# PolusAI/nyxus

Hardware: AMD Instinct MI355X
Metric: ROIs/sec (*ALL_GLCM*+*ALL_INTENSITY*, 1024^2 tiles) (higher is better)
Workload: dtype f64; 1 GPU; *ALL_GLCM*+*ALL_INTENSITY*, coarse_gray_depth=8, 4 angles, d=1, 1000 synthetic 1024x1024 tiles/GPU x 196 ROIs/tile (disk r=30, 2821 px, bbox 61x61), intensities U[1,4095]; reduce stage on pre-assembled ROI clouds resident in HBM; n_columns=185

## Files before the change

nyxus_amd/csrc/nyxhip_ctx.h:

```cpp
#pragma once
#include <hip/hip_runtime.h>
#include <math.h>
#include <stdio.h>
#include <stdlib.h>
#include <string.h>
#include <unistd.h>
#include <string>
#include <vector>
#include <algorithm>
#include <atomic>
#include <utility>

#include "../../include/nyxhip.h"
#include "roi_kernel.h"
#include "roi_radial.h"

struct DevBuf {
    void* p = nullptr;
    size_t bytes = 0;
    DevBuf() = default;
    DevBuf(const DevBuf&) = delete;
    DevBuf& operator=(const DevBuf&) = delete;
    DevBuf(DevBuf&& o) noexcept : p(o.p), bytes(o.bytes) { o.p = nullptr; o.bytes = 0; }
    DevBuf& operator=(DevBuf&& o) noexcept
// ... 65 lines not shown
};
constexpr int NYXHIP_INTERNAL_NEEDS_CLOUDS = -1000;

struct nyxhip_ctx {
    int device = 0;
    hipStream_t own_stream = nullptr;
    hipStream_t user_stream = nullptr;
    bool use_user_stream = false;
    DevBuf d_status;
    uint64_t census_small = 0, census_total = 0, census_pending = 0;
    DevBuf d_bank;
    DevBuf d_bank32;
    DevBuf d_bank16;
    std::vector<double> bank_key;
    uint32_t bank_zero_rows[NYXHIP_MAX_GABOR_FILTERS + 1] = {};
    uint32_t bank_lp_sep = 0;
    float bank_lp_B[16] = {}, bank_lp_C[44] = {};
    uint32_t bank_box_mask = 0;
    DevBuf d_stamps;
    std::string err;
    DevBuf d_stage;
    DevBuf d_glcm_ws;
    DevBuf d_glcm_ng;
    DevBuf d_logtab;
    uint32_t logtab_n = 0;
    DevBuf d_mom;
    DevBuf d_spill_list;
    DevBuf d_spill;
    DevBuf d_tile;
    DevBuf d_cloud;
    DevBuf d_slot[2];
    hipStream_t copy_stream = nullptr;
    hipEvent_t slot_ready[2] = {nullptr, nullptr}, slot_free[2] = {nullptr, nullptr};
    static constexpr int kStageSlots = 4;
    static constexpr size_t kStageSlotBytes = (size_t)32 << 20;
    PinnedSlot h_stage[kStageSlots];
    int h_stage_next = 0;
    nyxhip::WindowSrc win_next = {};
    uint32_t tile_cap_hint = 0;
    DevBuf d_res;
    size_t res_cap = 0, res_rows = 0, res_cols = 0;
    double* res_table() const { return d_res.as<double>(); }
    uint32_t* res_label() const { return (uint32_t*)(d_res.as<char>() + (((size_t)res_cap * res_cols * 8 + 255) & ~(size_t)255)); }
    uint32_t* res_tile() const { return res_label() + res_cap; }
    DevBuf d_cls_list;
    DevBuf d_cls_hdr;
// ... 53 lines not shown
```

nyxus_amd/csrc/nyxhip_dispatch.hip:

```cpp
#include "nyxhip_ctx.h"

using namespace nyxhip;

namespace {

uint32_t align16(uint32_t v) { return (v + 15u) & ~15u; }

void gabor_filter(double* Gex, double f0, double sig2lam, double gamma, double theta, double fi, int n)
{
    const double lambda = 2 * M_PI / f0, cos_theta = cos(theta), sin_theta = sin(theta), sig = sig2lam * lambda;
    std::vector<double> tx(n + 1), ty(n + 1);
    tx[0] = (n % 2 > 0) ? -((n - 1) / 2) : -(n / 2);
    for (int x = 1; x < n; x++) tx[x] = tx[x - 1] + 1;
    ty[0] = tx[0];
    for (int y = 1; y < n; y++) ty[y] = ty[y - 1] + 1;
    double sum = 0;
    for (int y = 0; y < n; y++)
        for (int x = 0; x < n; x++) {
            double xte = tx[x] * cos_theta + ty[y] * sin_theta;
            double yte = ty[y] * cos_theta - tx[x] * sin_theta;
            double rte = xte * xte + gamma * gamma * yte * yte;
            double ge = exp(-1 * rte / (2 * sig * sig));
            double argm = xte * f0 + fi;
            int idx = y * n * 2 + x * 2;
// ... 272 lines not shown
    int c_glrlm = n_cols1, c_gldzm = c_glrlm + ((mask & NYXHIP_FAM_GLRLM) ? kGlrlmCols : 0);
    int c_glszm = c_gldzm + ((mask & NYXHIP_FAM_GLDZM) ? kGldzmCols : 0), c_gldm = c_glszm + ((mask & NYXHIP_FAM_GLSZM) ? kGlszmCols : 0);
    int c_ngldm = c_gldm + ((mask & NYXHIP_FAM_GLDM) ? kGldmCols : 0);
    if (mask1 && (groups & 1)) {
        if (int lrc = make_layout(mask1, s, n_cols1, E.px, E.area, E.range, a.L, why, cap, E.vmax, E.wide_only))
            return lrc;
        a.n_roi = b->n_roi;
        a.px_offset = b->px_offset; a.x = b->x; a.y = b->y; a.inten = b->inten;
        a.bbox_w = b->bbox_w; a.bbox_h = b->bbox_h; a.min_inten = b->min_inten; a.max_inten = b->max_inten;
        a.slide_min = b->slide_min; a.slide_max = b->slide_max;
        a.out = d_out; a.ld = ld; a.status = ctx->d_status.as<int>();
        a.stamps = ctx->d_stamps.as<unsigned long long>();
        if (cap == 0) a.win = ctx->win_next;
        a.mask = mask1; a.n_cols = n_cols1;
        int c = 0;
        a.col_intensity = a.col_glcm = -1;
        if (mask1 & NYXHIP_FAM_INTENSITY) { a.col_intensity = c; c += kIntensityCols; }
        if (mask1 & NYXHIP_FAM_GLCM) { a.col_glcm = c; c += kGlcmAngled * s->glcm_n_angles + kGlcmAve; }
        a.soft_nan = s->soft_nan;
        a.grey_depth = s->grey_depth; a.ibsi = s->ibsi; a.glcm_grey_depth = s->glcm_grey_depth;
        a.glcm_offset = s->glcm_offset; a.glcm_na = s->glcm_n_angles; a.glcm_symmetric = s->glcm_symmetric;
        for (int i = 0; i < kMaxAngles; i++) a.glcm_angles[i] = s->glcm_angles[i];
        a.n_hist = abs(s->grey_depth);
        const int gi = s->ibsi ? 0 : s->grey_depth;
        if ((mask1 & NYXHIP_FAM_GLCM) && cap == 0 && gi >= 0 && a.L.ng_cap <= 16 && (int)a.L.app >= s->glcm_n_angles && s->glcm_n_angles > 0) {
            const size_t stride = (size_t)s->glcm_n_angles * a.L.ng_cap * a.L.ng_cap;
            const size_t need = 4 * stride * (size_t)b->n_roi + 256;
            if (ctx->d_glcm_ws.reserve(need, nullptr) != hipSuccess || !ctx->d_glcm_ng) {
                why = "out of device memory for the GLCM count workspace";
                return NYXHIP_ERR_HIP;
            }
            {
                a.glcm_ng = ctx->d_glcm_ng.as<uint32_t>();
                a.glcm_ws = ctx->d_glcm_ws.as<uint32_t>();
                a.glcm_ws_stride = (uint32_t)stride;
            }
        }
    }
    if (mask2 && (groups & 2)) {
        if (int lrc = make_tex_layout(mask2, s, n_cols2, E.area, E.side, t.L, why, cap, E.vmax))
            return lrc;
        t.n_roi = b->n_roi;
        t.px_offset = b->px_offset; t.x = b->x; t.y = b->y; t.inten = b->inten;
        t.bbox_w = b->bbox_w; t.bbox_h = b->bbox_h; t.min_inten = b->min_inten; t.max_inten = b->max_inten;
        t.out = d_out; t.ld = ld; t.status = ctx->d_status.as<int>();
        t.mask = mask2; t.n_cols = n_cols2; t.col0 = n_cols1;
// ... 740 lines not shown
        if (int brc = ensure_gabor_bank(ctx, s))
            return brc;
    hipStream_t st = ctx->stream();
    const uint32_t n_roi = (uint32_t)b->n_roi;
    clear_runs(ctx);
    if (!ctx->lane_fork) HIP_TRY(ctx, hipEventCreateWithFlags(&ctx->lane_fork, hipEventDisableTiming));
    HIP_TRY(ctx, hipEventRecord(ctx->lane_fork, st));
    struct LaneJoin {
        nyxhip_ctx* c; hipStream_t st;
        ~LaneJoin() {
            for (int k = 0; k < nyxhip_ctx::kLanes; k++)
                if (c->lane_used[k]) {
                    (void)hipEventRecord(c->lane_done[k], c->lane_stream[k]);
                    (void)hipStreamWaitEvent(st, c->lane_done[k], 0);
                    c->lane_used[k] = false;
                }
        }
    } lane_join{ctx, st};
    if (mask & NYXHIP_FAM_GLCM) {
        const size_t need = 4ull * n_roi + 256;
        HIP_TRY(ctx, ctx->d_glcm_ng.reserve(need, st, need + need / 4));
        HIP_TRY(ctx, hipMemsetAsync(ctx->d_glcm_ng.p, 0, 4ull * n_roi, st));
    }
    auto timed_class = [&](int cls, uint32_t count, const Extrema& E, const uint32_t* lp, uint32_t grid, uint32_t class_mask = 0, uint32_t group_sel = 0xF,
                           const ClassTotals* tot = nullptr) -> int {
        ClassRun r{cls, count, E, 0, nullptr, nullptr};
        if (ctx->timing >= 2) {
            HIP_TRY(ctx, hipEventCreate(&r.e0));
            HIP_TRY(ctx, hipEventCreate(&r.e1));
            HIP_TRY(ctx, hipEventRecord(r.e0, st));
        }
        const int rc = run_class(ctx, b, mask, s, d_out, ld, E, lp, grid, false, nullptr, &r, class_mask, group_sel, cls, tot);
        if (ctx->timing >= 2 && rc == 0) HIP_TRY(ctx, hipEventRecord(r.e1, st));
        ctx->runs.push_back(r);
        return rc;
    };
    if ((mask & ~kContourFams) || !hinted) {
        bool done = false;
        static const bool force_exact = [] { const char* e = getenv("NYXHIP_CLASS_SYNC"); return e && *e && *e != '0'; }();
        const bool need_vmax = s->ibsi && (mask & (NYXHIP_FAM_GLCM | kTexture | kDependence));
        const bool wide_possible = max_range >= 16384u && (mask & NYXHIP_FAM_INTENSITY);
        const bool has_m1 = !(max_px <= kClassPx[0] && max_side <= kClassSide[0]);
        static const bool no_small = [] { const char* e = getenv("NYXHIP_NO_SMALL"); return e && *e && *e != '0'; }();
        static const bool no_adapt = [] { const char* e = getenv("NYXHIP_NO_ADAPT"); return e && *e && *e != '0'; }();
        const bool small_fits = !no_small && ((mask & NYXHIP_FAM_INTENSITY) || (!s->ibsi && s->grey_depth > 0 && s->grey_depth <= 64));
        const bool two_filtered = (mask & (NYXHIP_FAM_INTENSITY | NYXHIP_FAM_GLCM)) && has_m1 && small_fits;
// ... 339 lines not shown
```

nyxus_amd/csrc/roi_features.hip:

```cpp
#include <hip/hip_runtime.h>
#include <type_traits>
#include <algorithm>
#include <cstdlib>
#include <cstdio>
#include "device_math.h"
#include "roi_kernel.h"
#include "launch_util.h"
#include "glcm_rows.h"
#include "glcm_w64.h"
#include "sort_lds.h"
#include "../../include/nyxhip.h"

namespace nyxhip {


enum { S_MEAN = 0, S_P10, S_P90, S_MEDIAN, S_MODE, S_NG };


template <int NW> __device__ __forceinline__ double xw_chain(const double* s_red, int k)
{
    return NW == 1 ? s_red[k] : ((s_red[k] + s_red[8 + k]) + s_red[16 + k]) + s_red[24 + k];
}
template <int NW> __device__ __forceinline__ double xw_pairs(const double* s_red, int k)
{
// ... 654 lines not shown
#define STAMP(i) do { } while (0)
#endif

typedef __attribute__((address_space(3))) uint8_t lds_u8_t;

typedef const __attribute__((address_space(4))) RoiArgs KArgs;
__device__ __forceinline__ KArgs* late_kernarg()
{
    KArgs* p = (KArgs*)__builtin_amdgcn_kernarg_segment_ptr();
    asm volatile("" : "+s"(p));
    return p;
}
template <bool LATE>
struct KView {
    const RoiArgs& a;
    KArgs* p;
    __device__ __forceinline__ explicit KView(const RoiArgs& a_) : a(a_), p(LATE ? late_kernarg() : nullptr) {}
    __device__ __forceinline__ auto operator->() const
    {
        if constexpr (LATE) return p;
        else return &a;
    }
};
template <bool GS, bool C16, bool SPLIT, bool D8, int FAM = 0, int TIER = 4, bool G16 = false, int WIN = 2, int NW = 4>
__device__ __forceinline__ void roi_features_body(const RoiArgs& A, const uint64_t slot)
{
    static_assert((NW == 4 && NW == kMaxAngles) || (NW == 8 && G16 && FAM == 4), "one workgroup of four waves per ROI (and a wave per GLCM angle)");
    constexpr int BS = NW * 64;
    extern __shared__ __attribute__((aligned(16))) unsigned char lds_raw[];
    unsigned char* const lds = GS ? A.sp.scratch + (size_t)blockIdx.x * A.sp.stride : lds_raw;
    const int tid = (int)threadIdx.x, lane = tid & 63, wave = __builtin_amdgcn_readfirstlane(tid >> 6);
    uint64_t roi;
    if (!roi_of_slot(A.sp, slot, A.n_roi, roi))
        return;

    auto reg = [&](uint32_t o) -> unsigned char* { return (GS && o < A.L.gs_lds_bytes) ? lds_raw + o : lds + o; };
    double* s_red = (double*)reg(A.L.red);
    double* s_stat = (double*)reg(A.L.stat);
    uint32_t* s_lb100 = (uint32_t*)reg(A.L.lb100);
    uint32_t* s_lbc = (uint32_t*)reg(A.L.lbc);
    uint32_t* s_val = (uint32_t*)(lds + A.L.val);
    using dense_t = typename std::conditional<D8, uint8_t, uint16_t>::type;
    dense_t* s_dense = (dense_t*)(lds + (D8 ? 0u : A.L.dense));
    uint16_t* s_lvlmap = (uint16_t*)reg(A.L.lvlmap);
    uint32_t* s_P = (uint32_t*)reg(A.L.P);
    double* s_g = (double*)reg(A.L.gscr);

// ... 314 lines not shown
    }

    STAMP(1);
    const KView<FAM != 0 || G16> B(A);
    double* const out_row_l = B->out + roi * B->ld;
    if (do_int) {
        double* o = out_row_l + B->col_intensity;
        const double dn = (double)n;
        if ((unsigned long long)n * vmax < (1ull << 32))
            sum = wave_sum_t<uint32_t>((uint32_t)sum);
        else
            sum = wave_sum_u64(sum);
        if (C16) {
            const uint32_t lo24 = wave_sum_t<uint32_t>((uint32_t)sumsq & 0xFFFFFFu), hi = wave_sum_t<uint32_t>((uint32_t)(sumsq >> 24));
            sumsq = ((unsigned long long)hi << 24) + lo24;
        } else
            sumsq = wave_sum_u64(sumsq);
        if (lane == 0) {
            s_red[wave * 8 + 0] = (double)sum;
            s_red[wave * 8 + 1] = (double)sumsq;
        }
        grp_sync<GS, NW>();
        const bool blank = (vmin == 0 && vmax == 0);
        if (tid == 0) {
            double tot = 0, totsq = 0;
            for (int wv = 0; wv < NW; wv++) {
                tot += s_red[wv * 8 + 0];
                totsq += s_red[wv * 8 + 1];
            }
            const double mean = tot / dn;
            s_stat[S_MEAN] = mean;
            if (FAST)
                s_stat[S_NG] = bin_pixel(vmin, vmin, vmax, B->glcm_grey_depth) == bin_pixel(vmax, vmin, vmax, B->glcm_grey_depth) ? 1.0 : 0.0;
            o[I_MIN] = (double)vmin;
            o[I_MAX] = (double)vmax;
            o[I_RANGE] = (double)vmax - (double)vmin;
            if (B->slide_min && B->slide_max)
                o[I_COVERED_IMAGE_INTENSITY_RANGE] = (double)(vmax - vmin) / (B->slide_max[roi] - B->slide_min[roi]);
            o[I_MEAN] = mean;
            o[I_ENERGY] = totsq;
            o[I_ROOT_MEAN_SQUARED] = sqrt(totsq / dn);
            o[I_INTEGRATED_INTENSITY] = tot;
            if (!blank)
                o[I_UNIFORMITY_PIU] = (1.0 - (double)(vmax - vmin) / (double)(uint32_t)(vmax + vmin)) * 100.0;
        }
        grp_sync<GS, NW>();
        const double mean = s_stat[S_MEAN];
        STAMP(2);

        const double binW100 = (double)range / 100.;
        const uint32_t nb = (uint32_t)B->n_hist;
        auto idx100 = [=](uint32_t v) -> int {
            double realIdx = (double)(v - vmin) / binW100;
            return (realIdx != realIdx) ? 0 : (int)realIdx;
        };

        const uint32_t Q = ((range + 1 + NW * 512 - 1) / (NW * 512)) * 512;
        uint32_t* const s_woff = (uint32_t*)(s_stat + 8);
        if (use_count) {
            uint32_t carry = 0, best_c = 0, best_i = 0;
            const uint32_t base = wave * Q;
            if (C16) {
                uint32_t kk[8] = {0, 0, 0, 0, 0, 0, 0, 0};
                uint32_t inv = 0xFFFFu - (base + 8u * (uint32_t)lane);
                uint4* src = (uint4*)((uint16_t*)s_cnt + base + 8u * (uint32_t)lane);
                uint32_t i = base + 8u * (uint32_t)lane;
                for (uint32_t t = 0; t < Q; t += 512, i += 512, inv -= 512, src += 64) {
// ... 240 lines not shown
                for (int q = 0; q < 6; q++) {
                    const double frac = q == 0 ? 0.01 : q == 1 ? 0.1 : q == 2 ? 0.25 : q == 3 ? 0.75 : q == 4 ? 0.9 : 0.99;
                    const double cnt_p = dn * frac;
                    bool m0 = (double)r0 <= cnt_p && cnt_p <= (double)e0;
                    bool m1 = i1 < 100 && (double)r1 <= cnt_p && cnt_p <= (double)e1;
                    unsigned long long b0 = __ballot(m0), b1 = __ballot(m1);
                    int win = b1 ? 64 + (63 - __clzll((long long)b1)) : (b0 ? 63 - __clzll((long long)b0) : -1);
                    if (lane == q) { mywin = win; mycnt = cnt_p; }
                }
                double pv = 0;
                if (mywin >= 0) {
                    uint32_t rs = s_lb100[mywin], bi = (mywin < 99 ? s_lb100[mywin + 1] : n) - rs;
                    pv = (mycnt - (double)rs) * binW100 / (double)bi + (double)vmin + binW100 * (double)mywin;
                }
                double pq[6];
#pragma unroll
                for (int q = 0; q < 6; q++) {
                    const unsigned long long u = (unsigned long long)__double_as_longlong(pv);
                    const uint32_t lo = (uint32_t)__builtin_amdgcn_readlane((int)(uint32_t)u, q), hi = (uint32_t)__builtin_amdgcn_readlane((int)(uint32_t)(u >> 32), q);
                    pq[q] = __longlong_as_double((long long)(((unsigned long long)hi << 32) | lo));
                }
                if (lane == 0) {
                    o[I_P01] = pq[0]; o[I_P10] = pq[1]; o[I_P25] = pq[2]; o[I_P75] = pq[3]; o[I_P90] = pq[4]; o[I_P99] = pq[5];
                    o[I_QCOD] = (pq[3] - pq[2]) / (pq[3] + pq[2]);
                    o[I_INTERQUARTILE_RANGE] = pq[3] - pq[2];
                    s_stat[S_P10] = pq[1];
                    s_stat[S_P90] = pq[4];
                    if (FUSED) {
                        const double p10 = pq[1], p90 = pq[4];
                        uint32_t lox = 0x80000000u, span = 0;
                        if (p10 <= p90 && p90 >= (double)vmin && p10 <= (double)vmax) {
                            const double cl = ceil(p10), fl = floor(p90);
                            const uint32_t lo_v = cl <= (double)vmin ? vmin : (uint32_t)cl, hi_v = fl >= (double)vmax ? vmax : (uint32_t)fl;
                            if (lo_v <= hi_v) { lox = lo_v - vmin; span = hi_v - lo_v; }
                        }
                        const bool empty = span == 0 && lox == 0x80000000u;
                        uint32_t* const s_rob = (uint32_t*)(s_stat + 6);
                        s_rob[0] = lox;
                        s_rob[1] = span;
                        s_rob[2] = (empty || lox == 0) ? 0u : cum(lox - 1);
                        s_rob[3] = empty ? 0u : cum(lox + span);
                    }
                }
            }
            if (NW == 1 || wave == 1) {
                double e = 0, u = 0;
                for (uint32_t k = lane; k < nb; k += 64) {
                    uint32_t ck = (k < nb - 1 ? s_lbc[k + 1] : n) - s_lbc[k];
// ... 79 lines not shown
                    px1(pv[n_full * BS]);
                {
                    const uint32_t wsx = wave_sum_t<uint32_t>(sx), wsad = wave_sum_t<uint32_t>(sad);
                    if (lane == 0) {
                        s_red[wave * 8 + 6] = (double)wsx;
                        s_red[wave * 8 + 7] = (double)wsad;
                    }
                }
                {
                    double t[8];
#pragma unroll
                    for (int k = 0; k < 8; k++) t[k] = k < 6 ? acc[k] : 0.0;
                    const double tot = wave_transpose_sum8(t, lane);
                    if ((lane & 7) == 0 && (lane >> 3) < 6)
                        s_red[wave * 8 + (lane >> 3)] = tot;
                }
                grp_sync<GS, NW>();
                const uint32_t n_below = (uint32_t)__builtin_amdgcn_readfirstlane((int)s_rob[2]);
                const uint32_t n_upto = (uint32_t)__builtin_amdgcn_readfirstlane((int)s_rob[3]);
                const uint32_t K = n_upto - n_below, n_above = n - n_upto;
                const uint32_t Sx_all = (uint32_t)xw_pairs<NW>(s_red, 6);
                const uint32_t Sxu = (uint32_t)__builtin_amdgcn_readfirstlane((int)(Sx_all - n_below * lox - n_above * hix));
                const double Sx = (double)Sxu, dK = (double)K;
                if (tid == 0) {
                    double a6[6];
#pragma unroll
                    for (int k = 0; k < 6; k++) {
                        a6[k] = xw_chain<NW>(s_red, k);
                        asm volatile("" : "+v"(a6[k]) :: "memory");
                    }
                    const double sadk = xw_pairs<NW>(s_red, 7);
                    const double sadt = 2.0 * sadk + ((m2x & 1u) ? 2.0 * (double)((const uint32_t*)(s_stat + 10))[1] - dn : 0.0);
                    central_outputs(a6);
                    o[I_ROBUST_MEAN] = K ? (Sx + dK * (double)vmin) / dK : 0.0;
                    o[I_MEDIAN_ABSOLUTE_DEVIATION] = fdiv(sadt * 0.5, dn);
                }
                const uint32_t Ku = K;
                const bool fast32 = (unsigned long long)(n_full + 1) * Ku * (span + 1ull) < (1ull << 32);
                double ad1[1];
                if (fast32) {
                    uint32_t ad = 0;
                    auto px2 = [&](uint32_t x) {
                        const uint32_t t = mul_u24_su(med3_u32_ss(x, lox, hix), Ku);
                        asm("v_sad_u32 %0, %1, %2, %0" : "+v"(ad) : "v"(t), "s"(Sxu));
                    };
                    {
                        uint32_t k = 0;
                        for (; k + 1 < n_full; k += 2) { px2(pv[k * BS]); px2(pv[(k + 1) * BS]); }
                        if (k < n_full) px2(pv[k * BS]);
                    }
                    if ((uint32_t)tid < n_rem)
                        px2(pv[n_full * BS]);
                    ad1[0] = (double)ad;
                } else {
                    unsigned long long ad = 0;
                    auto px2 = [&](uint32_t x) {
                        const uint32_t t = (uint32_t)__umul24(Ku, x);
                        uint32_t dlt;
                        asm("v_sad_u32 %0, %1, %2, 0" : "=v"(dlt) : "v"(t), "s"(Sxu));
                        ad += (x - lox) <= span ? dlt : 0u;
                    };
                    for (uint32_t k = 0; k < n_full; k++)
                        px2(pv[k * BS]);
                    if ((uint32_t)tid < n_rem)
                        px2(pv[n_full * BS]);
                    ad1[0] = (double)ad;
                }
                block_sum<1, GS, NW>(ad1, (double*)s_lb100, tid);
                if (tid == 0) {
                    double adin = ad1[0];
                    if (fast32) {
                        const double klo = (double)Ku * (double)lox, khi = (double)Ku * (double)hix;
                        adin -= (double)n_below * fabs(klo - Sx) + (double)n_above * fabs(khi - Sx);
                    }
                    o[I_ROBUST_MEAN_ABSOLUTE_DEVIATION] = K ? fdiv(fdiv(adin, dK), dK) : 0.0;
                }
            } else {
            double rb[3] = {0, 0, 0};
            for (uint32_t i = tid; i < n; i += BS) {
                double a = (double)(C16 ? vmin + ((const uint16_t*)s_val)[i] : SV(i));
                if (a >= p10 && a <= p90) {
                    rb[0] += a;
                    rb[1] += 1.0;
                }
                rb[2] += fabs(a - median);
            }
            block_sum<3, GS, NW>(rb, s_red, tid);
            const double mean1090 = rb[1] > 0 ? rb[0] / rb[1] : 0.0;
            double ad[1] = {0};
            for (uint32_t i = tid; i < n; i += BS) {
                double a = (double)(C16 ? vmin + ((const uint16_t*)s_val)[i] : SV(i));
// ... 144 lines not shown
#pragma unroll
                    for (int q = 0; q < kMaxAngles; q++) {
                        if (q >= na)
                            break;
                        const int ang = B->glcm_angles[q];
                        const int dx = ang == 90 ? 0 : ang == 135 ? -B->glcm_offset : B->glcm_offset, dy = ang == 0 ? 0 : B->glcm_offset;
                        const int r2 = row + dy, c2 = col + dx;
                        if (r2 < 0 || r2 >= (int)h || c2 < 0 || c2 >= (int)w)
                            continue;
                        const uint32_t la = s_dense[(uint32_t)r2 * w + (uint32_t)c2];
                        if (la == 0)
                            continue;
                        atomicAdd(&s_P[q * NN + ((int)lb - 1) * Ng + (int)la - 1], 1u);
                        if (symmetric)
                            atomicAdd(&s_P[q * NN + ((int)la - 1) * Ng + (int)lb - 1], 1u);
                    }
                }
        }
        grp_sync<GS, NW>();
        STAMP(11);
        {
            uint32_t* dst = B->glcm_ws + roi * B->glcm_ws_stride;
            if (dpp) {
                const float inv_nn = __builtin_amdgcn_rcpf((float)NN), inv_ng = __builtin_amdgcn_rcpf((float)Ng);
                for (int i = tid; i < na * NN; i += BS) {
                    const uint32_t q = (uint32_t)(((float)i + 0.5f) * inv_nn), rem = (uint32_t)i - mul24(q, (uint32_t)NN);
                    const uint32_t r = (uint32_t)(((float)rem + 0.5f) * inv_ng), c = rem - mul24(r, (uint32_t)Ng);
                    dst[i] = s_P[mad24(q, (uint32_t)cells, mad24(r + 1u, (uint32_t)NG1, c + 1u))];
                }
            } else
                for (int i = tid; i < na * NN; i += BS)
                    dst[i] = s_P[i];
        }
        STAMP(12);
    } else
    if (do_glcm) {
        double* o = out_row_l + B->col_glcm;
        const int na = B->glcm_na;
        const int ncol_g = kGlcmAngled * na + kGlcmAve;
        const uint32_t vmin_g = (uint32_t)__builtin_amdgcn_readfirstlane((int)vmin), vmax_g = (uint32_t)__builtin_amdgcn_readfirstlane((int)vmax);
        const bool degenerate = bin_pixel(vmin_g, vmin_g, vmax_g, B->glcm_grey_depth) == bin_pixel(vmax_g, vmin_g, vmax_g, B->glcm_grey_depth);

        double* s_I = s_g;
        double* s_f = s_g + B->L.ng_cap;
        double* s_scr = s_f + kMaxAngles * 32;
        if (FAST) {
        } else if (greyInfo > 0) {
            if (tid == 0)
                s_stat[S_NG] = (double)greyInfo;
        } else {
            lvl_max = wave_max_u32(lvl_max);
// ... 514 lines not shown
__global__ __launch_bounds__(kBlock, 4) void roi_features_kernel(const RoiArgs A)
{
    roi_features_body<GS, C16, SPLIT, D8>(A, blockIdx.x);
}

template <bool C16, bool SPLIT, bool D8>
__global__ __launch_bounds__(kBlock, 5) void roi_features_kernel_occ5(const RoiArgs A)
{
    roi_features_body<false, C16, SPLIT, D8, 0, 5>(A, blockIdx.x);
}
template <bool C16, bool SPLIT, bool D8>
__global__ __launch_bounds__(kBlock, 6) void roi_features_kernel_occ6(const RoiArgs A)
{
    roi_features_body<false, C16, SPLIT, D8, 0, 6>(A, blockIdx.x);
}
template <bool C16, bool SPLIT, bool D8>
__global__ __launch_bounds__(kBlock, 7) void roi_features_kernel_occ7(const RoiArgs A)
{
    roi_features_body<false, C16, SPLIT, D8, 0, 7>(A, blockIdx.x);
}
template <int FAM, int WIN>
__global__ __launch_bounds__(kBlock, 8) void roi_features_kernel_occ8(const RoiArgs A)
{
    roi_features_body<false, true, FAM == 1 || FAM == 3, true, FAM, 8, false, WIN>(A, (WIN == 1 && A.win.xcd_swz) ? xcd_slot(blockIdx.x, gridDim.x) : (uint64_t)blockIdx.x);
}
template <int FAM, int WIN>
__global__ __launch_bounds__(kBlock, 7) void roi_features_kernel_fam7(const RoiArgs A)
{
    roi_features_body<false, true, FAM == 1 || FAM == 3, true, FAM, 7, false, WIN>(A, (WIN == 1 && A.win.xcd_swz) ? xcd_slot(blockIdx.x, gridDim.x) : (uint64_t)blockIdx.x);
}
template <int FAM, int WIN>
__global__ __launch_bounds__(kBlock, 6) void roi_features_kernel_fam6(const RoiArgs A)
{
    roi_features_body<false, true, FAM == 1 || FAM == 3, true, FAM, 6, false, WIN>(A, (WIN == 1 && A.win.xcd_swz) ? xcd_slot(blockIdx.x, gridDim.x) : (uint64_t)blockIdx.x);
}

template <int WIN>
__global__ __launch_bounds__(kBlock, 4) void roi_features_kernel_g16(const RoiArgs A)
{
    roi_features_body<false, true, false, true, 0, 9, true, WIN>(A, (WIN == 1 && A.win.xcd_swz) ? xcd_slot(blockIdx.x, gridDim.x) : (uint64_t)blockIdx.x);
}

template <int WIN>
__global__ __launch_bounds__(512, 8) void roi_features_kernel_g16w8(const RoiArgs A)
{
    roi_features_body<false, true, false, true, 4, 9, true, WIN, 8>(A, (WIN == 1 && A.win.xcd_swz) ? xcd_slot(blockIdx.x, gridDim.x) : (uint64_t)blockIdx.x);
}
// ... 98 lines not shown
    for (int q = 0; q < 2; q++) {
        if (Ng[q] == 0) continue;
        double* o = A.out + roi[q] * A.ld + A.col_glcm;
        const double* fq = (const double*)(base + (size_t)q * cnt_bytes);
        for (int c = lane; c < kGlcmAngled * na; c += 64) {
            const int k = sh >= 0 ? c >> sh : c / na, a = c - k * na;
            o[c] = fq[a * 32 + k];
        }
        for (int j = lane; j < kGlcmAve; j += 64) {
            const int k = c_glcm_ave_order[j];
            double init = 0.0;
            int a = 0;
            for (; na - a >= 4; a += 4) {
                const double v1 = fq[a * 32 + k] + fq[(a + 1) * 32 + k];
                const double v2 = fq[(a + 2) * 32 + k] + fq[(a + 3) * 32 + k];
                init = init + (v1 + v2);
            }
            for (; a < na; a++) init = init + fq[a * 32 + k];
            o[kGlcmAngled * na + j] = na == 4 ? init * 0.25 : na == 2 ? init * 0.5 : na ? init / (double)na : 0.0;
        }
    }
}

size_t glcm_features8_lds(uint32_t ng_cap)
{
    return (2 * glcm8_cnt_bytes(ng_cap) + 8ull * (2 * kMaxAngles * 16 + 2 * kMaxAngles * 32)) * kWaves;
}

size_t glcm_features_lds(uint32_t ng_cap)
{
    const size_t per_wave = (((size_t)4 * kMaxAngles * ng_cap * ng_cap + 15) & ~(size_t)15) + 8ull * (ng_cap + kMaxAngles * 6 * ng_cap + 2 * kMaxAngles * 32);
    return per_wave * kWaves;
}

size_t roi_features_max_lds()
{
    return 160 * 1024;
}

namespace {

int no_static_lds(const void* f)
{
    hipFuncAttributes at;
    if (hipError_t e = hipFuncGetAttributes(&at, f); e != hipSuccess)
        return (int)e;
    return at.sharedSizeBytes == 0 ? 0 : (int)hipErrorInvalidConfiguration;
}

template <bool C16, bool SPLIT, bool D8>
int launch_lds_variant(const RoiArgs& a, hipStream_t st, uint32_t grid)
{
    static DeviceOnce optin;
    if (int orc = optin.run([]() -> int {
        const void* fns[22] = {(const void*)roi_features_kernel<false, C16, SPLIT, D8>, (const void*)roi_features_kernel_occ5<C16, SPLIT, D8>,
                               (const void*)roi_features_kernel_occ6<C16, SPLIT, D8>, (const void*)roi_features_kernel_occ7<C16, SPLIT, D8>,
                               (const void*)roi_features_kernel_occ8<1, 0>, (const void*)roi_features_kernel_occ8<2, 0>,
                               (const void*)roi_features_kernel_occ8<1, 1>, (const void*)roi_features_kernel_occ8<2, 1>,
                               (const void*)roi_features_kernel_fam7<1, 0>, (const void*)roi_features_kernel_fam7<2, 0>,
                               (const void*)roi_features_kernel_fam7<1, 1>, (const void*)roi_features_kernel_fam7<2, 1>,
                               (const void*)roi_features_kernel_fam6<1, 0>, (const void*)roi_features_kernel_fam6<2, 0>,
                               (const void*)roi_features_kernel_fam6<1, 1>, (const void*)roi_features_kernel_fam6<2, 1>,
                               (const void*)roi_features_kernel_occ8<3, 0>, (const void*)roi_features_kernel_occ8<3, 1>,
                               (const void*)roi_features_kernel_fam7<3, 0>, (const void*)roi_features_kernel_fam7<3, 1>,
                               (const void*)roi_features_kernel_fam6<3, 0>, (const void*)roi_features_kernel_fam6<3, 1>};
        for (const void* f : fns) {
            hipError_t e = hipFuncSetAttribute(f, hipFuncAttributeMaxDynamicSharedMemorySize, (int)roi_features_max_lds());
            if (e != hipSuccess)
                return (int)e;
            if (int src = no_static_lds(f))
                return src;
        }
        return 0;
    }))
        return orc;
    const size_t lds = roi_features_max_lds();
    const bool int_only = !(a.mask & NYXHIP_FAM_GLCM) && (a.mask & NYXHIP_FAM_INTENSITY);
    const bool int_glcm = (a.mask & NYXHIP_FAM_GLCM) && (a.mask & NYXHIP_FAM_INTENSITY) && a.L.dense8 && a.glcm_ws != nullptr && !a.ibsi &&
                          a.grey_depth > 0 && a.grey_depth <= 16;
    const bool glcm_only = (a.mask & NYXHIP_FAM_GLCM) && !(a.mask & NYXHIP_FAM_INTENSITY) && a.L.dense8 && a.glcm_ws != nullptr && !a.ibsi &&
                           a.grey_depth > 0 && a.grey_depth <= 16;
    const bool fam_ok = C16 && SPLIT && D8 && (int_only || int_glcm || glcm_only);
    int occ = 4;
    for (int o = fam_ok ? 8 : 7; o > 4; o--)
        if ((size_t)o * a.L.total <= lds) { occ = o; break; }
    if (const char* e = getenv("NYXHIP_MAX_OCC")) occ = occ < atoi(e) ? occ : (atoi(e) < 4 ? 4 : atoi(e));
    const bool win = a.win.inten != nullptr;
    if (win && a.win.xcd_swz) grid = (grid + 7u) & ~7u;
    if (fam_ok && glcm_only && occ >= 6) {
        if (occ == 8) { if (win) hipLaunchKernelGGL((roi_features_kernel_occ8<3, 1>), dim3(grid), dim3(kBlock), a.L.total, st, a);
                        else hipLaunchKernelGGL((roi_features_kernel_occ8<3, 0>), dim3(grid), dim3(kBlock), a.L.total, st, a); }
        else if (occ == 7) { if (win) hipLaunchKernelGGL((roi_features_kernel_fam7<3, 1>), dim3(grid), dim3(kBlock), a.L.total, st, a);
                             else hipLaunchKernelGGL((roi_features_kernel_fam7<3, 0>), dim3(grid), dim3(kBlock), a.L.total, st, a); }
        else { if (win) hipLaunchKernelGGL((roi_features_kernel_fam6<3, 1>), dim3(grid), dim3(kBlock), a.L.total, st, a);
               else hipLaunchKernelGGL((roi_features_kernel_fam6<3, 0>), dim3(grid), dim3(kBlock), a.L.total, st, a); }
    }
    else if (occ == 8 && int_only && win) hipLaunchKernelGGL((roi_features_kernel_occ8<2, 1>), dim3(grid), dim3(kBlock), a.L.total, st, a);
    else if (occ == 8 && int_only) hipLaunchKernelGGL((roi_features_kernel_occ8<2, 0>), dim3(grid), dim3(kBlock), a.L.total, st, a);
    else if (occ == 8 && win) hipLaunchKernelGGL((roi_features_kernel_occ8<1, 1>), dim3(grid), dim3(kBlock), a.L.total, st, a);
    else if (occ == 8) hipLaunchKernelGGL((roi_features_kernel_occ8<1, 0>), dim3(grid), dim3(kBlock), a.L.total, st, a);
    else if (fam_ok && occ == 7 && int_only && win) hipLaunchKernelGGL((roi_features_kernel_fam7<2, 1>), dim3(grid), dim3(kBlock), a.L.total, st, a);
    else if (fam_ok && occ == 7 && int_only) hipLaunchKernelGGL((roi_features_kernel_fam7<2, 0>), dim3(grid), dim3(kBlock), a.L.total, st, a);
    else if (fam_ok && occ == 7 && win) hipLaunchKernelGGL((roi_features_kernel_fam7<1, 1>), dim3(grid), dim3(kBlock), a.L.total, st, a);
    else if (fam_ok && occ == 7) hipLaunchKernelGGL((roi_features_kernel_fam7<1, 0>), dim3(grid), dim3(kBlock), a.L.total, st, a);
    else if (fam_ok && occ == 6 && int_only && win) hipLaunchKernelGGL((roi_features_kernel_fam6<2, 1>), dim3(grid), dim3(kBlock), a.L.total, st, a);
    else if (fam_ok && occ == 6 && int_only) hipLaunchKernelGGL((roi_features_kernel_fam6<2, 0>), dim3(grid), dim3(kBlock), a.L.total, st, a);
    else if (fam_ok && occ == 6 && win) hipLaunchKernelGGL((roi_features_kernel_fam6<1, 1>), dim3(grid), dim3(kBlock), a.L.total, st, a);
    else if (fam_ok && occ == 6) hipLaunchKernelGGL((roi_features_kernel_fam6<1, 0>), dim3(grid), dim3(kBlock), a.L.total, st, a);
    else if (occ == 7) hipLaunchKernelGGL((roi_features_kernel_occ7<C16, SPLIT, D8>), dim3(grid), dim3(kBlock), a.L.total, st, a);
    else if (occ == 6) hipLaunchKernelGGL((roi_features_kernel_occ6<C16, SPLIT, D8>), dim3(grid), dim3(kBlock), a.L.total, st, a);
    else if (occ == 5) hipLaunchKernelGGL((roi_features_kernel_occ5<C16, SPLIT, D8>), dim3(grid), dim3(kBlock), a.L.total, st, a);
// ... 23 lines not shown
                for (const void* f : {(const void*)roi_features_kernel_g16<0>, (const void*)roi_features_kernel_g16<1>,
                                      (const void*)roi_features_kernel_g16w8<0>, (const void*)roi_features_kernel_g16w8<1>}) {
                    if (hipError_t e = hipFuncSetAttribute(f, hipFuncAttributeMaxDynamicSharedMemorySize, (int)roi_features_max_lds()); e != hipSuccess)
                        return (int)e;
                    if (int src = no_static_lds(f))
                        return src;
                }
                return 0;
            }))
            return orc;
        static const bool w4 = [] { const char* e = getenv("NYXHIP_G16_W4"); return e && *e && *e != '0'; }();
        static const uint32_t g16_w8_min = [] { const char* e = getenv("NYXHIP_G16_W8_MIN"); return e && *e ? (uint32_t)atoi(e) : 48u * 48u; }();
        if (!(a.mask & NYXHIP_FAM_INTENSITY) && !w4 && a.L.dense_cap >= g16_w8_min) {
            if (a.win.inten != nullptr) hipLaunchKernelGGL(roi_features_kernel_g16w8<1>, dim3(a.win.xcd_swz ? (grid + 7u) & ~7u : grid), dim3(512), a.L.total, st, a);
            else hipLaunchKernelGGL(roi_features_kernel_g16w8<0>, dim3(grid), dim3(512), a.L.total, st, a);
        } else
        if (a.win.inten != nullptr) hipLaunchKernelGGL(roi_features_kernel_g16<1>, dim3(a.win.xcd_swz ? (grid + 7u) & ~7u : grid), dim3(kBlock), a.L.total, st, a);
        else hipLaunchKernelGGL(roi_features_kernel_g16<0>, dim3(grid), dim3(kBlock), a.L.total, st, a);
        return (int)hipGetLastError();
    }
    const bool split = a.glcm_ws != nullptr;
    const bool d8 = a.L.dense8 != 0 || (c16 && !(a.mask & NYXHIP_FAM_GLCM));
    int rc;
    if (a.small_class && !no_small && (c16 || !(a.mask & NYXHIP_FAM_INTENSITY)) && roi_small_supported(a)) rc = launch_roi_small(a, st, grid, a.small_class == 2);
    else
    rc = d8 ? launch_lds_variant<true, true, true>(a, st, grid)
           : c16 ? (split ? launch_lds_variant<true, true, false>(a, st, grid) : launch_lds_variant<true, false, false>(a, st, grid))
                 : (split ? launch_lds_variant<false, true, false>(a, st, grid) : launch_lds_variant<false, false, false>(a, st, grid));
    if (rc == 0 && split && a.glcm_feats != 1) {
        static const bool no_pairs = [] { const char* e = getenv("NYXHIP_GLCM_NO_PAIRS"); return e && *e && *e != '0'; }();
        RoiArgs af = a;
        if (a.glcm_feats == 2) af.sp.class_mask = 0;
        if (a.L.ng_cap <= 8 && !no_pairs)
            hipLaunchKernelGGL(glcm_features_kernel8, dim3((grid + 2 * kWaves - 1) / (2 * kWaves)), dim3(kBlock), glcm_features8_lds(a.L.ng_cap), st, af);
        else
            hipLaunchKernelGGL(glcm_features_kernel, dim3((grid + kWaves - 1) / kWaves), dim3(kBlock), glcm_features_lds(a.L.ng_cap), st, af);
        rc = (int)hipGetLastError();
    }
    return rc;
}

}
```

nyxus_amd/csrc/roi_kernel.h:

```cpp
#pragma once
#include <stdint.h>
#include <stddef.h>
#include "../../include/nyxhip.h"

namespace nyxhip {

constexpr int kBlock = 256;
constexpr int kWaves = kBlock / 64;
constexpr int kIntensityCols = 36;
constexpr int kGlcmAngled = 30;
constexpr int kGlcmAve = 29;
constexpr int kMaxAngles = 4;

constexpr int kSizeClasses = 5, kClasses = 2 * kSizeClasses;
constexpr uint32_t kClassPx[kSizeClasses - 1] = {256, 4096, 16384, 32768};
constexpr uint32_t kClassSide[kSizeClasses - 1] = {32, 64, 128, 256};
constexpr uint32_t kLdsLevels = 128;
constexpr int kFirstLargeSizeClass = 3;
__host__ __device__ inline int roi_class(uint32_t n, uint32_t w, uint32_t h, uint32_t range, uint32_t lvl = 0)
{
    const uint32_t side = w > h ? w : h;
    int sc = (n <= 256u && side <= 32u) ? 0 : (n <= 4096u && side <= 64u) ? 1 : (n <= 16384u && side <= 128u) ? 2 : (n <= 32768u && side <= 256u) ? 3 : 4;
    if (sc == 2 && range >= 65536u) sc = 3;
    if (sc < 3 && lvl > kLdsLevels) sc = 3;
// ... 49 lines not shown
    uint32_t dense_cap;
    uint32_t ng_cap;
    uint32_t lvl_cap;
    uint32_t app;
    uint32_t g16;
    uint32_t gs_lds_bytes;
    uint32_t radix;
    uint32_t radix_k16;
};

struct WindowSrc {
    const void* inten;
    const void* lab;
    int32_t dt_inten, dt_label;
    uint32_t W, H;
    const uint32_t* tile;
    const uint32_t* label;
    const uint32_t* x0;
    const uint32_t* y0;
    uint32_t xcd_swz;
};
__host__ __device__ inline uint64_t xcd_slot(uint32_t b, uint32_t grid) { const uint32_t per = (grid + 7u) >> 3; return (uint64_t)(b & 7u) * per + (b >> 3); }

struct RoiArgs {
    uint64_t n_roi;
    const uint64_t* px_offset;
    const uint16_t* x;
    const uint16_t* y;
    const uint32_t* inten;
    const uint32_t* bbox_w;
    const uint32_t* bbox_h;
    const uint32_t* min_inten;
    const uint32_t* max_inten;
    const double* slide_min;
    const double* slide_max;
    double* out;
    uint64_t ld;
    int* status;
    unsigned long long* stamps;
    uint32_t mask;
    int32_t n_cols;
    int32_t col_intensity;
    int32_t col_glcm;
    double soft_nan;
    int32_t grey_depth, ibsi, glcm_grey_depth, glcm_offset, glcm_na, glcm_symmetric;
    int32_t glcm_angles[kMaxAngles];
    int32_t n_hist;
    uint32_t* glcm_ws;
    uint32_t* glcm_ng;
    uint32_t glcm_ws_stride;
    uint32_t* census;
    uint32_t small_class;
    uint32_t glcm_feats;
    SpillArgs sp;
    WindowSrc win;
    LdsLayout L;
};

constexpr int kGlrlmCols = 16 * 4 + 16;
constexpr int kGlszmCols = 16;
constexpr int kNgtdmCols = 5;

constexpr int kRlmLdsCols = 16;
struct TexLayout {
    uint32_t out;
    uint32_t red;
    uint32_t stat;
    uint32_t dense;
    uint32_t lvlmap;
    uint32_t lv;
    uint32_t lvf;
    uint32_t work;
    uint32_t total;
    uint32_t dense_cap, side_cap, lvl_cap, ng_cap, hash_cap, work_bytes, szm_ok;
    uint32_t szm_c16;
    uint32_t szm_small, szm_smalltab;
// ... 402 lines not shown
```

Measured before the change: 96.99 million ROIs/s.

## Defer intensity feature finalization to a separate close kernel with coalesced writes

In the occupancy-8 fused ROI kernel, intensity scalar epilogues (moments, robust stats, QCOD) are no longer computed and written per ROI. Instead the raw accumulators go into a compact per-ROI record, and a new 64-lane close kernel finishes the math and writes the columns, staged through LDS so stores are spread across lanes. This is meant to shorten the serial tid==0 tail in the main kernel and cut its register and store pressure. The cost is an extra launch plus record and flag traffic. Separately, the GLCM workspace copy uses shift and mask indexing when Ng is a power of two, replacing float reciprocal division.

```diff
diff --git a/nyxus_amd/csrc/nyxhip_ctx.h b/nyxus_amd/csrc/nyxhip_ctx.h
--- a/nyxus_amd/csrc/nyxhip_ctx.h
+++ b/nyxus_amd/csrc/nyxhip_ctx.h
@@ -111,6 +111,8 @@
     DevBuf d_stage;
     DevBuf d_glcm_ws;
     DevBuf d_glcm_ng;
+    DevBuf d_close_rec;
+    DevBuf d_close_flag;
     DevBuf d_logtab;
     uint32_t logtab_n = 0;
     DevBuf d_mom;
diff --git a/nyxus_amd/csrc/nyxhip_dispatch.hip b/nyxus_amd/csrc/nyxhip_dispatch.hip
--- a/nyxus_amd/csrc/nyxhip_dispatch.hip
+++ b/nyxus_amd/csrc/nyxhip_dispatch.hip
@@ -318,6 +318,10 @@
         a.glcm_offset = s->glcm_offset; a.glcm_na = s->glcm_n_angles; a.glcm_symmetric = s->glcm_symmetric;
         for (int i = 0; i < kMaxAngles; i++) a.glcm_angles[i] = s->glcm_angles[i];
         a.n_hist = abs(s->grey_depth);
+        if ((mask1 & NYXHIP_FAM_INTENSITY) && cap == 0) {
+            a.close_rec = ctx->d_close_rec.as<double>();
+            a.close_flag = ctx->d_close_flag.as<uint32_t>();
+        }
         const int gi = s->ibsi ? 0 : s->grey_depth;
         if ((mask1 & NYXHIP_FAM_GLCM) && cap == 0 && gi >= 0 && a.L.ng_cap <= 16 && (int)a.L.app >= s->glcm_n_angles && s->glcm_n_angles > 0) {
             const size_t stride = (size_t)s->glcm_n_angles * a.L.ng_cap * a.L.ng_cap;
@@ -1104,6 +1108,12 @@
         HIP_TRY(ctx, ctx->d_glcm_ng.reserve(need, st, need + need / 4));
         HIP_TRY(ctx, hipMemsetAsync(ctx->d_glcm_ng.p, 0, 4ull * n_roi, st));
     }
+    if (mask & NYXHIP_FAM_INTENSITY) {
+        const size_t need_rec = 8ull * kCloseRec * n_roi + 256, need_flag = 4ull * n_roi + 256;
+        HIP_TRY(ctx, ctx->d_close_rec.reserve(need_rec, st, need_rec + need_rec / 4));
+        HIP_TRY(ctx, ctx->d_close_flag.reserve(need_flag, st, need_flag + need_flag / 4));
+        HIP_TRY(ctx, hipMemsetAsync(ctx->d_close_flag.p, 0, 4ull * n_roi, st));
+    }
     auto timed_class = [&](int cls, uint32_t count, const Extrema& E, const uint32_t* lp, uint32_t grid, uint32_t class_mask = 0, uint32_t group_sel = 0xF,
                            const ClassTotals* tot = nullptr) -> int {
         ClassRun r{cls, count, E, 0, nullptr, nullptr};
diff --git a/nyxus_amd/csrc/roi_features.hip b/nyxus_amd/csrc/roi_features.hip
--- a/nyxus_amd/csrc/roi_features.hip
+++ b/nyxus_amd/csrc/roi_features.hip
@@ -700,7 +700,7 @@
         else return &a;
     }
 };
-template <bool GS, bool C16, bool SPLIT, bool D8, int FAM = 0, int TIER = 4, bool G16 = false, int WIN = 2, int NW = 4>
+template <bool GS, bool C16, bool SPLIT, bool D8, int FAM = 0, int TIER = 4, bool G16 = false, int WIN = 2, int NW = 4, bool DEFER_P = false>
 __device__ __forceinline__ void roi_features_body(const RoiArgs& A, const uint64_t slot)
 {
     static_assert((NW == 4 && NW == kMaxAngles) || (NW == 8 && G16 && FAM == 4), "one workgroup of four waves per ROI (and a wave per GLCM angle)");
@@ -1061,6 +1061,13 @@
         }
         grp_sync<GS, NW>();
         const bool blank = (vmin == 0 && vmax == 0);
+#if defined(NYX_NO_FUSED) || defined(NYX_NO_DEFER)
+        constexpr bool DEFER = false;
+#else
+        constexpr bool DEFER = DEFER_P && C16 && !GS;
+#endif
+        const bool defer = DEFER && !blank;
+        double* const rec = DEFER ? B->close_rec + roi * kCloseRec : nullptr;
         if (tid == 0) {
             double tot = 0, totsq = 0;
             for (int wv = 0; wv < NW; wv++) {
@@ -1071,6 +1078,10 @@
             s_stat[S_MEAN] = mean;
             if (FAST)
                 s_stat[S_NG] = bin_pixel(vmin, vmin, vmax, B->glcm_grey_depth) == bin_pixel(vmax, vmin, vmax, B->glcm_grey_depth) ? 1.0 : 0.0;
+            if (defer) {
+                rec[CR_TOT] = tot;
+                rec[CR_TOTSQ] = totsq;
+            } else {
             o[I_MIN] = (double)vmin;
             o[I_MAX] = (double)vmax;
             o[I_RANGE] = (double)vmax - (double)vmin;
@@ -1082,6 +1093,7 @@
             o[I_INTEGRATED_INTENSITY] = tot;
             if (!blank)
                 o[I_UNIFORMITY_PIU] = (1.0 - (double)(vmax - vmin) / (double)(uint32_t)(vmax + vmin)) * 100.0;
+            }
         }
         grp_sync<GS, NW>();
         const double mean = s_stat[S_MEAN];
@@ -1368,8 +1380,10 @@
                 }
                 if (lane == 0) {
                     o[I_P01] = pq[0]; o[I_P10] = pq[1]; o[I_P25] = pq[2]; o[I_P75] = pq[3]; o[I_P90] = pq[4]; o[I_P99] = pq[5];
-                    o[I_QCOD] = (pq[3] - pq[2]) / (pq[3] + pq[2]);
-                    o[I_INTERQUARTILE_RANGE] = pq[3] - pq[2];
+                    if (!DEFER) {
+                        o[I_QCOD] = (pq[3] - pq[2]) / (pq[3] + pq[2]);
+                        o[I_INTERQUARTILE_RANGE] = pq[3] - pq[2];
+                    }
                     s_stat[S_P10] = pq[1];
                     s_stat[S_P90] = pq[4];
                     if (FUSED) {
@@ -1495,6 +1509,15 @@
                 const uint32_t Sx_all = (uint32_t)xw_pairs<NW>(s_red, 6);
                 const uint32_t Sxu = (uint32_t)__builtin_amdgcn_readfirstlane((int)(Sx_all - n_below * lox - n_above * hix));
                 const double Sx = (double)Sxu, dK = (double)K;
+                if (DEFER) {
+                    if (tid < 8)
+                        rec[CR_ACC + tid] = xw_chain<NW>(s_red, tid);
+                    if (tid == 0) {
+                        uint32_t* const rw = (uint32_t*)rec;
+                        *(uint4*)(rw + CR_W_NBELOW) = make_uint4(n_below, n_above, K, Sxu);
+                        *(uint4*)(rw + CR_W_LOX) = make_uint4(lox, hix, m2x, ((const uint32_t*)(s_stat + 10))[1]);
+                    }
+                } else
                 if (tid == 0) {
                     double a6[6];
 #pragma unroll
@@ -1540,6 +1563,13 @@
                     ad1[0] = (double)ad;
                 }
                 block_sum<1, GS, NW>(ad1, (double*)s_lb100, tid);
+                if (DEFER) {
+                    if (tid == 0) {
+                        rec[CR_ADIN] = ad1[0];
+                        ((uint32_t*)rec)[CR_W_FAST32] = fast32 ? 1u : 0u;
+                        B->close_flag[roi] = 1u;
+                    }
+                } else
                 if (tid == 0) {
                     double adin = ad1[0];
                     if (fast32) {
@@ -1730,11 +1760,21 @@
         {
             uint32_t* dst = B->glcm_ws + roi * B->glcm_ws_stride;
             if (dpp) {
+                if ((Ng & (Ng - 1)) == 0 && ((na * NN) & (BS - 1)) == 0) {
+                    const int lg = 31 - __builtin_clz((unsigned)Ng);
+                    const uint32_t cm = (uint32_t)Ng - 1u;
+                    for (int i0 = 0; i0 < na * NN; i0 += BS) {
+                        const uint32_t i = (uint32_t)(i0 + tid);
+                        const uint32_t q = i >> (2 * lg), r = (i >> lg) & cm, c = i & cm;
+                        dst[i] = s_P[mad24(q, (uint32_t)cells, mad24(r + 1u, (uint32_t)NG1, c + 1u))];
+                    }
+                } else {
                 const float inv_nn = __builtin_amdgcn_rcpf((float)NN), inv_ng = __builtin_amdgcn_rcpf((float)Ng);
                 for (int i = tid; i < na * NN; i += BS) {
                     const uint32_t q = (uint32_t)(((float)i + 0.5f) * inv_nn), rem = (uint32_t)i - mul24(q, (uint32_t)NN);
                     const uint32_t r = (uint32_t)(((float)rem + 0.5f) * inv_ng), c = rem - mul24(r, (uint32_t)Ng);
                     dst[i] = s_P[mad24(q, (uint32_t)cells, mad24(r + 1u, (uint32_t)NG1, c + 1u))];
+                }
                 }
             } else
                 for (int i = tid; i < na * NN; i += BS)
@@ -2295,7 +2335,7 @@
 template <int FAM, int WIN>
 __global__ __launch_bounds__(kBlock, 8) void roi_features_kernel_occ8(const RoiArgs A)
 {
-    roi_features_body<false, true, FAM == 1 || FAM == 3, true, FAM, 8, false, WIN>(A, (WIN == 1 && A.win.xcd_swz) ? xcd_slot(blockIdx.x, gridDim.x) : (uint64_t)blockIdx.x);
+    roi_features_body<false, true, FAM == 1 || FAM == 3, true, FAM, 8, false, WIN, 4, FAM == 1 || FAM == 2>(A, (WIN == 1 && A.win.xcd_swz) ? xcd_slot(blockIdx.x, gridDim.x) : (uint64_t)blockIdx.x);
 }
 template <int FAM, int WIN>
 __global__ __launch_bounds__(kBlock, 7) void roi_features_kernel_fam7(const RoiArgs A)
@@ -2440,6 +2480,137 @@
     }
 }
 
+constexpr int kCloseBlock = 64;
+constexpr uint64_t kCloseCols =
+    (1ull << I_MIN) | (1ull << I_MAX) | (1ull << I_RANGE) | (1ull << I_COVERED_IMAGE_INTENSITY_RANGE) | (1ull << I_MEAN) | (1ull << I_ENERGY) |
+    (1ull << I_ROOT_MEAN_SQUARED) | (1ull << I_INTEGRATED_INTENSITY) | (1ull << I_UNIFORMITY_PIU) | (1ull << I_MEAN_ABSOLUTE_DEVIATION) |
+    (1ull << I_VARIANCE) | (1ull << I_VARIANCE_BIASED) | (1ull << I_STANDARD_DEVIATION) | (1ull << I_STANDARD_DEVIATION_BIASED) | (1ull << I_COV) |
+    (1ull << I_STANDARD_ERROR) | (1ull << I_SKEWNESS) | (1ull << I_KURTOSIS) | (1ull << I_EXCESS_KURTOSIS) | (1ull << I_HYPERSKEWNESS) |
+    (1ull << I_HYPERFLATNESS) | (1ull << I_ROBUST_MEAN) | (1ull << I_MEDIAN_ABSOLUTE_DEVIATION) | (1ull << I_ROBUST_MEAN_ABSOLUTE_DEVIATION) |
+    (1ull << I_QCOD) | (1ull << I_INTERQUARTILE_RANGE);
+__global__ __launch_bounds__(kCloseBlock) void intensity_close_kernel(const RoiArgs A)
+{
+    constexpr int kPitch = __builtin_popcountll(kCloseCols);
+#ifndef NYX_CLOSE_DIRECT
+    __shared__ double s_o[kCloseBlock * kPitch];
+#endif
+    const int lane = (int)threadIdx.x;
+    uint64_t roi = 0;
+    bool mine = roi_of_slot(A.sp, (uint64_t)blockIdx.x * kCloseBlock + (uint64_t)lane, A.n_roi, roi) && glcm_roi_in_launch(A, roi);
+    if (mine) mine = A.close_flag[roi] != 0;
+    const unsigned long long todo = __ballot(mine);
+    if (todo == 0)
+        return;
+#ifdef NYX_CLOSE_DIRECT
+    double* const o = A.out + roi * A.ld + A.col_intensity;
+    auto O = [&](int c) -> double& { return o[c]; };
+#else
+    double* const o = s_o + lane * kPitch;
+    auto O = [&](int c) -> double& { return o[__builtin_popcountll(kCloseCols & ((1ull << c) - 1ull))]; };
+#endif
+    if (mine) {
+        A.close_flag[roi] = 0;
+        const double* const rec = A.close_rec + roi * kCloseRec;
+        const uint32_t* const rw = (const uint32_t*)rec;
+        const double* const row = A.out + roi * A.ld + A.col_intensity;
+        const uint32_t n = (uint32_t)(A.px_offset[roi + 1] - A.px_offset[roi]);
+        const uint32_t vmin = A.min_inten[roi], vmax = A.max_inten[roi];
+        const double2 s01 = *(const double2*)(rec + CR_TOT);
+        double acc[6];
+#pragma unroll
+        for (int k = 0; k < 6; k += 2) {
+            const double2 t = *(const double2*)(rec + CR_ACC + k);
+            acc[k] = t.x; acc[k + 1] = t.y;
+        }
+        const double sadk = rec[CR_SADK], adin0 = rec[CR_ADIN];
+        const bool fast32 = rw[CR_W_FAST32] != 0;
+        const uint4 w0 = *(const uint4*)(rw + CR_W_NBELOW), w1 = *(const uint4*)(rw + CR_W_LOX);
+        const uint32_t n_below = w0.x, n_above = w0.y, K = w0.z, Sxu = w0.w, lox = w1.x, hix = w1.y, m2x = w1.z, cle = w1.w;
+        const double p25 = row[I_P25], p75 = row[I_P75];
+#pragma unroll
+        for (int c = 0; c < kIntensityCols; c++)
+            if ((kCloseCols >> c) & 1ull) O(c) = 0.0;
+        const double dn = (double)n;
+        constexpr bool blank = false;
+        const double tot = s01.x, totsq = s01.y;
+        const double mean = tot / dn;
+        O(I_MIN) = (double)vmin;
+        O(I_MAX) = (double)vmax;
+        O(I_RANGE) = (double)vmax - (double)vmin;
+        if (A.slide_min && A.slide_max)
+            O(I_COVERED_IMAGE_INTENSITY_RANGE) = (double)(vmax - vmin) / (A.slide_max[roi] - A.slide_min[roi]);
+        O(I_MEAN) = mean;
+        O(I_ENERGY) = totsq;
+        O(I_ROOT_MEAN_SQUARED) = sqrt(totsq / dn);
+        O(I_INTEGRATED_INTENSITY) = tot;
+        if (!blank)
+            O(I_UNIFORMITY_PIU) = (1.0 - (double)(vmax - vmin) / (double)(uint32_t)(vmax + vmin)) * 100.0;
+        {
+            const double var = acc[1];
+            const double inv_n = frcp(dn);
+            O(I_MEAN_ABSOLUTE_DEVIATION) = acc[0] * inv_n;
+            const double variance = dn > 1 ? var * frcp(dn - 1) : 0.0;
+            const double variance_b = dn > 1 ? var * inv_n : 0.0;
+            const double rsd = variance > 0 ? frsq(variance) : 0.0;
+            const double sd = variance * rsd;
+            const double rs_n = frsq(dn);
+            O(I_VARIANCE) = variance;
+            O(I_VARIANCE_BIASED) = variance_b;
+            O(I_STANDARD_DEVIATION) = sd;
+            O(I_STANDARD_DEVIATION_BIASED) = variance_b > 0 ? variance_b * frsq(variance_b) : 0.0;
+            O(I_COV) = sd / mean;
+            O(I_STANDARD_ERROR) = sd * rs_n;
+            if (!blank) {
+                const double M2 = acc[1], M3 = acc[2], M4 = acc[3];
+                if (M2 != 0.0) {
+                    const double r = frsq(M2), r2 = r * r;
+                    const double kurt = n > 4 ? (dn * M4) * (r2 * r2) : 0.0;
+                    O(I_SKEWNESS) = n > 3 ? ((dn * rs_n) * M3) * (r2 * r) : 0.0;
+                    O(I_KURTOSIS) = kurt;
+                    O(I_EXCESS_KURTOSIS) = n > 4 ? kurt - 3 : 0.0;
+                }
+                const double rsd2 = rsd * rsd, t5 = inv_n * (rsd2 * rsd2 * rsd);
+                O(I_HYPERSKEWNESS) = acc[4] * t5;
+                O(I_HYPERFLATNESS) = acc[5] * (t5 * rsd);
+            }
+        }
+        {
+            const double Sx = (double)Sxu, dK = (double)K;
+            const double sadt = 2.0 * sadk + ((m2x & 1u) ? 2.0 * (double)cle - dn : 0.0);
+            O(I_ROBUST_MEAN) = K ? (Sx + dK * (double)vmin) / dK : 0.0;
+            O(I_MEDIAN_ABSOLUTE_DEVIATION) = fdiv(sadt * 0.5, dn);
+            const uint32_t Ku = K;
+            double adin = adin0;
+            if (fast32) {
+                const double klo = (double)Ku * (double)lox, khi = (double)Ku * (double)hix;
+                adin -= (double)n_below * fabs(klo - Sx) + (double)n_above * fabs(khi - Sx);
+            }
+            O(I_ROBUST_MEAN_ABSOLUTE_DEVIATION) = K ? fdiv(fdiv(adin, dK), dK) : 0.0;
+        }
+        O(I_QCOD) = (p75 - p25) / (p75 + p25);
+        O(I_INTERQUARTILE_RANGE) = p75 - p25;
+    }
+#ifndef NYX_CLOSE_DIRECT
+    __syncthreads();
+    int mycol = -1;
+    {
+        int rank = 0;
+#pragma unroll
+        for (int c = 0; c < kIntensityCols; c++)
+            if ((kCloseCols >> c) & 1ull) { if (rank == lane) mycol = c; rank++; }
+    }
+    const uint32_t roi_lo = (uint32_t)roi, roi_hi = (uint32_t)(roi >> 32);
+    double* const dst0 = A.out + A.col_intensity + (mycol >= 0 ? mycol : 0);
+#pragma unroll 8
+    for (int r = 0; r < kCloseBlock; r++) {
+        if (!((todo >> r) & 1ull)) continue;
+        const uint64_t rr = ((uint64_t)(uint32_t)__builtin_amdgcn_readlane((int)roi_hi, r) << 32) | (uint32_t)__builtin_amdgcn_readlane((int)roi_lo, r);
+        if (mycol >= 0)
+            dst0[rr * A.ld] = s_o[r * kPitch + lane];
+    }
+#endif
+}
+
 size_t glcm_features8_lds(uint32_t ng_cap)
 {
     return (2 * glcm8_cnt_bytes(ng_cap) + 8ull * (2 * kMaxAngles * 16 + 2 * kMaxAngles * 32)) * kWaves;
@@ -2467,8 +2638,9 @@
 }
 
 template <bool C16, bool SPLIT, bool D8>
-int launch_lds_variant(const RoiArgs& a, hipStream_t st, uint32_t grid)
-{
+int launch_lds_variant(const RoiArgs& a, hipStream_t st, uint32_t grid, bool& deferred)
+{
+    deferred = false;
     static DeviceOnce optin;
     if (int orc = optin.run([]() -> int {
         const void* fns[22] = {(const void*)roi_features_kernel<false, C16, SPLIT, D8>, (const void*)roi_features_kernel_occ5<C16, SPLIT, D8>,
@@ -2505,6 +2677,13 @@
     if (const char* e = getenv("NYXHIP_MAX_OCC")) occ = occ < atoi(e) ? occ : (atoi(e) < 4 ? 4 : atoi(e));
     const bool win = a.win.inten != nullptr;
     if (win && a.win.xcd_swz) grid = (grid + 7u) & ~7u;
+#if defined(NYX_NO_FUSED) || defined(NYX_NO_DEFER)
+    deferred = false;
+#else
+    deferred = occ == 8 && (a.mask & NYXHIP_FAM_INTENSITY) != 0;
+#endif
+    if (deferred && !(a.close_rec && a.close_flag))
+        return (int)hipErrorInvalidValue;
     if (fam_ok && glcm_only && occ >= 6) {
         if (occ == 8) { if (win) hipLaunchKernelGGL((roi_features_kernel_occ8<3, 1>), dim3(grid), dim3(kBlock), a.L.total, st, a);
                         else hipLaunchKernelGGL((roi_features_kernel_occ8<3, 0>), dim3(grid), dim3(kBlock), a.L.total, st, a); }
@@ -2574,11 +2753,16 @@
     const bool split = a.glcm_ws != nullptr;
     const bool d8 = a.L.dense8 != 0 || (c16 && !(a.mask & NYXHIP_FAM_GLCM));
     int rc;
+    bool deferred = false;
     if (a.small_class && !no_small && (c16 || !(a.mask & NYXHIP_FAM_INTENSITY)) && roi_small_supported(a)) rc = launch_roi_small(a, st, grid, a.small_class == 2);
     else
-    rc = d8 ? launch_lds_variant<true, true, true>(a, st, grid)
-           : c16 ? (split ? launch_lds_variant<true, true, false>(a, st, grid) : launch_lds_variant<true, false, false>(a, st, grid))
-                 : (split ? launch_lds_variant<false, true, false>(a, st, grid) : launch_lds_variant<false, false, false>(a, st, grid));
+    rc = d8 ? launch_lds_variant<true, true, true>(a, st, grid, deferred)
+           : c16 ? (split ? launch_lds_variant<true, true, false>(a, st, grid, deferred) : launch_lds_variant<true, false, false>(a, st, grid, deferred))
+                 : (split ? launch_lds_variant<false, true, false>(a, st, grid, deferred) : launch_lds_variant<false, false, false>(a, st, grid, deferred));
+    if (rc == 0 && deferred) {
+        hipLaunchKernelGGL(intensity_close_kernel, dim3((grid + kCloseBlock - 1) / kCloseBlock), dim3(kCloseBlock), 0, st, a);
+        rc = (int)hipGetLastError();
+    }
     if (rc == 0 && split && a.glcm_feats != 1) {
         static const bool no_pairs = [] { const char* e = getenv("NYXHIP_GLCM_NO_PAIRS"); return e && *e && *e != '0'; }();
         RoiArgs af = a;
diff --git a/nyxus_amd/csrc/roi_kernel.h b/nyxus_amd/csrc/roi_kernel.h
--- a/nyxus_amd/csrc/roi_kernel.h
+++ b/nyxus_amd/csrc/roi_kernel.h
@@ -95,6 +95,17 @@
 };
 __host__ __device__ inline uint64_t xcd_slot(uint32_t b, uint32_t grid) { const uint32_t per = (grid + 7u) >> 3; return (uint64_t)(b & 7u) * per + (b >> 3); }
 
+constexpr int kCloseRec = 16;
+enum {
+    CR_TOT = 0, CR_TOTSQ,
+    CR_ACC,
+    CR_SADK = 9,
+    CR_ADIN,
+    CR_W_FAST32 = 22,
+    CR_W_NBELOW = 24, CR_W_NABOVE, CR_W_K, CR_W_SXU,
+    CR_W_LOX, CR_W_HIX, CR_W_M2X, CR_W_CLE
+};
+
 struct RoiArgs {
     uint64_t n_roi;
     const uint64_t* px_offset;
@@ -125,6 +136,8 @@
     uint32_t* census;
     uint32_t small_class;
     uint32_t glcm_feats;
+    double* close_rec;
+    uint32_t* close_flag;
     SpillArgs sp;
     WindowSrc win;
     LdsLayout L;
```

Result: faster. 99.70 million ROIs/s (median of 6 runs) (+2.8%).
